# mitroitskii/crosscoder-model-diff-replication

Hardware: AMD Instinct MI355X
Metric: activations/sec per train step (fwd+bwd+Adam), 2x2304->16384; % bf16 MFMA peak (higher is better)
Workload: dtype bf16; 1 GPU; crosscoder train step 2x2304->16384, batch 4096; global_batch=4096, n_models=2, d_model=2304, dict_size=16384, parallelism=latent1

## Files before the change

crosscoder-model-diff-replication_amd/_lib.py:

```python
import contextlib
import ctypes
import os

_HERE = os.path.dirname(os.path.abspath(__file__))
LIB_PATH = os.path.join(_HERE, "libcrosscoder_hip.so")
DEBUG_LIB_PATH = os.path.join(_HERE, "libcrosscoder_hip_dbg.so")
DEFAULT_PP_MASK = 7
_INT_SETTERS = ("cc_debug_set_pp_mask", "cc_debug_set_pp_fast", "cc_debug_set_dec_one_launch",
                "cc_debug_set_wave_sync", "cc_debug_set_epi_store", "cc_debug_set_q4", "cc_debug_set_adam_ref")
DEBUG_SETTERS = _INT_SETTERS + ("cc_debug_adam_prims", "cc_debug_adam_redone")

CC_BF16 = 1
CC_F32 = 2
CC_LAYOUT_KC = 0
CC_LAYOUT_MN = 1

_p = ctypes.c_void_p


class LossTailJob(ctypes.Structure):
    _fields_ = [("colsum_acts", ctypes.c_void_p), ("tn", ctypes.c_void_p), ("h", ctypes.c_int64),
                ("l1_part", ctypes.c_void_p), ("row_part", ctypes.c_void_p), ("ncb", ctypes.c_int64),
                ("l0_part", ctypes.c_void_p), ("n_l0", ctypes.c_int64), ("ev", ctypes.c_void_p),
                ("ev_a", ctypes.c_void_p), ("ev_b", ctypes.c_void_p), ("scalars", ctypes.c_void_p),
                ("l1l0_out", ctypes.c_void_p), ("host_out", ctypes.c_void_p), ("seq", ctypes.c_uint32),
                ("B", ctypes.c_int64), ("n", ctypes.c_int64), ("counter", ctypes.c_void_p)]


class ColsumJob(ctypes.Structure):
    _fields_ = [("part", ctypes.c_void_p), ("rows", ctypes.c_int64), ("cols", ctypes.c_int64), ("ld", ctypes.c_int64),
                ("scale", ctypes.c_float), ("out", ctypes.c_void_p)]
_i64 = ctypes.c_int64
_i = ctypes.c_int
_f = ctypes.c_float
_d = ctypes.c_double

SIGNATURES = {
    "cc_version": (_i, []),
    "cc_strerror": (ctypes.c_char_p, [_i]),
    "cc_col_part_rows": (_i64, [_i64]),
    "cc_wave_parts": (_i64, [_i64, _i64]),
    "cc_wgrad_parts": (_i64, [_i64, _i64, _i]),
    "cc_prep_part_rows": (_i64, [_i64]),
    "cc_loss_part_rows": (_i64, [_i64]),
    "cc_loss_col_blocks": (_i64, [_i64]),
    "cc_loss_scalars_len": (_i64, [_i64]),
# ... 52 lines not shown
                                    ctypes.c_double, _i64, _i64, _p, _p, _i, _p]),
    "cc_gather_rows": (_i, [_p, _i64, _p, _p, _i64, _i64, _p]),
    "cc_fold_scaling": (_i, [_p, _p, _p, _p, _i64, _i64, _i64, _i, _p]),
    "cc_decoder_stats": (_i, [_p, _i64, _i64, _i64, _i, _p, _p, _p, _p]),
    "cc_latent_stats_max_k": (_i, []),
    "cc_latent_stats_update": (_i, [_p, _i64, _i64, _i64, _i, _p, _i64, _i, _p, _p, _p, _p, _p, _p]),
    "cc_topk_part_rows": (_i64, [_i64, _i64]),
    "cc_topk_l0_parts": (_i64, [_i64, _i64]),
    "cc_topk_rows": (_i, [_p, _i64, _i64, _i64, _i, _i, _p, _p, _p, _p, _p, _p]),
    "cc_batch_topk_part_rows": (_i64, [_i64, _i64]),
    "cc_batch_topk_l0_parts": (_i64, [_i64, _i64]),
    "cc_batch_topk_ws_bytes": (_i64, [_i64, _i64, _i, _i]),
    "cc_batch_topk": (_i, [_p, _i64, _i64, _i64, _i, _p, _i64, _p, _p, _p, _p, _p, _p, _f, _p, _i64, _p]),
    "cc_threshold_mask": (_i, [_p, _i64, _i64, _i64, _i, _p, _p, _p, _p, _p, _p, _p]),
    "cc_adam_step": (_i, [_p, _p, _p, _p, _i64, _p, _d, _d, _d, _d, _i64, _i64, _i, _p]),
    "cc_adam_step_clip": (_i, [_p, _p, _p, _p, _i64, _p, _i, _f, _i, _p, _d, _d, _d, _d, _i64, _i64, _i, _p]),
    "cc_adam_dec_norms": (_i, [_p, _p, _p, _p, _i64, _p, _p, _i, _f, _i, _d, _d, _d, _d, _i64, _i64, _p, _i64, _i64, _i,
                               _p, _p]),
    "cc_adam_capped_blocks": (_i64, [_i64, _i64]),
    "cc_auxk_rows": (_i, [_p, _i64, _i64, _i64, _i, _i, _p, _i64, _p, _p, _p]),
    "cc_dead_update": (_i, [_p, _p, _i64, _i64, _i64, _i64, _p, _p, _p, _p]),
    "cc_auxk_part_floats": (_i64, [_i64, _i64]),
    "cc_auxk_loss": (_i, [_p, _p, _p, _p, _p, _p, _p, _p, _f, _i64, _i64, _i, _p]),
    "cc_add_rows": (_i, [_p, _p, _i64, _i64, _i64, _i, _p]),
    "cc_jumprelu_part_rows": (_i64, [_i64, _i64]),
    "cc_jumprelu_l0_parts": (_i64, [_i64, _i64]),
    "cc_jumprelu_mask": (_i, [_p, _i64, _i64, _i64, _i, _p, _f, _p, _p, _p, _p, _p]),
    "cc_jumprelu_bwd": (_i, [_p, _p, _i64, _i64, _i64, _i, _p, _f, _f, _p, _p, _p]),
}

# ... 78 lines not shown
```

crosscoder-model-diff-replication_amd/buffer.py:

```python
import numpy as np
import torch
import torch.distributed as dist
import tqdm

from . import ops
from .crosscoder import DTYPES



def _coll_device(group, default):
    if dist.get_backend(group) == "nccl":
        return torch.device("cuda", torch.cuda.current_device())
    return default


def _src(group, r):
    return dist.get_global_rank(group, r) if group is not None and group != dist.group.WORLD else r


def fingerprint(buf, factor):
    words = buf.reshape(buf.shape[0], -1).view(torch.int16)
    rows = words.shape[0]
    total = torch.zeros((), dtype=torch.int64, device=buf.device)
    step = 4096
# ... 110 lines not shown
            spare = torch.empty_like(self.buffer)
        self.gather_rows(self.buffer, perm, out=spare)
        self._spare, self.buffer = self.buffer, spare
        self.refresh_count += 1

    def next_raw(self):
        B = self.cfg["batch_size"]
        out = self.buffer[self.buffer_pointer: self.buffer_pointer + B]
        self.buffer_pointer += B
        if self.buffer_pointer > self.buffer.shape[0] // 2 - B:
            if out.dtype != torch.float32:
                out = out.clone()
            self.refresh()
        return out, self.normalisation_factor


class SyntheticBuffer(_BufferProtocol):

    RAW_SCALES = (1 / 0.2759, 1 / 0.2442, 1 / 0.31, 1 / 0.27)

    def __init__(self, cfg, rows, n_models=2, seed=0, device=None):
        device = device or cfg["device"]
        self.cfg = cfg
        self.dtype = DTYPES[cfg["enc_dtype"]]
        d = cfg["d_in"]
        g = torch.Generator(device=device).manual_seed(seed)
        scales = torch.tensor([self.RAW_SCALES[i % 4] for i in range(n_models)], device=device)
        buf = torch.empty(rows, n_models, d, dtype=self.dtype, device=device)
        chunk = 65536
        for r0 in range(0, rows, chunk):
# ... 1 lines not shown
            z = torch.randn(r1 - r0, n_models, d, generator=g, device=device)
            buf[r0:r1] = (z * scales[None, :, None]).to(self.dtype)
        self.buffer = buf
        sample = buf[: min(rows, 4096)].float()
        f = [(d ** 0.5) / sample[:, i].norm(dim=-1).mean().item() for i in range(n_models)]
        self.normalisation_factor = torch.tensor(f, device=device, dtype=self.dtype)
        self.buffer_pointer = 0

    def next_raw(self):
        B = self.cfg["batch_size"]
        if self.buffer_pointer + B > self.buffer.shape[0]:
            self.buffer_pointer = 0
        out = self.buffer[self.buffer_pointer: self.buffer_pointer + B]
        self.buffer_pointer += B
        return out, self.normalisation_factor
```

crosscoder-model-diff-replication_amd/csrc/step_kernels.hip:

```cpp
#include "cc_common.h"

#include <cfloat>
#include <cmath>

namespace cc {

#include "grad_tail.h"

constexpr int PREP_ROWS = 64;
constexpr int LOSS_ROWS = 32;
constexpr int LOSS_COLS = 512;

typedef __attribute__((address_space(3))) bf16x4 lds_bf16x4_s;
CC_DEV void tile_put8(char* lds, int r, int chunk, const float v[8]) {
  bf16x8 b;
#pragma unroll
  for (int j = 0; j < 8; ++j) b[j] = (short)f2bf(v[j]);
  *(bf16x8*)(lds + r * 1024 + ((chunk ^ (r & 7)) << 4)) = b;
}
template <int R, bool NT = false>
CC_DEV void tile_store_transposed(const char* lds, void* out_t, int64_t ldt, int64_t col0, int ncols, int64_t row0,
                                  int nrows) {
  constexpr int RQ = R / 32;
  const int lane = threadIdx.x & 63, wave = threadIdx.x >> 6;
  const int g = lane >> 4, i = lane & 15, q = i >> 2, p = i & 3;
  for (int it = wave; it < 32 * RQ; it += 4) {
    const int cg = it / RQ, rb = (it % RQ) * 32 + g * 8;
    const int ca = cg * 16 + 4 * p, c = cg * 16 + i;
    const int l0 = rb + q, l1 = rb + 4 + q;
    const bf16x4 v0 = __builtin_amdgcn_ds_read_tr16_b64_v4i16(
        (lds_bf16x4_s*)(lds + l0 * 1024 + (((ca >> 3) ^ (l0 & 7)) << 4) + (ca & 4) * 2));
    const bf16x4 v1 = __builtin_amdgcn_ds_read_tr16_b64_v4i16(
        (lds_bf16x4_s*)(lds + l1 * 1024 + (((ca >> 3) ^ (l1 & 7)) << 4) + (ca & 4) * 2));
    if (c < ncols && rb < nrows) {
      const bf16x8 v = bf16x8{v0[0], v0[1], v0[2], v0[3], v1[0], v1[1], v1[2], v1[3]};
      bf16x8* dst = (bf16x8*)((bf16_t*)out_t + (col0 + c) * ldt + row0 + rb);
      if constexpr (NT) __builtin_nontemporal_store(v, dst);
      else *dst = v;
    }
  }
}

template <int DIN, int DF, int DT, bool TR = false>
__global__ __launch_bounds__(256) void prep_kernel(const void* __restrict__ x_in, const void* __restrict__ factor,
                                                   void* __restrict__ x_out, float* __restrict__ colsum_part, int B,
                                                   int n, int d, void* __restrict__ x_t) {
  __shared__ __attribute__((aligned(16))) char lds[TR ? 32 * 1024 : 4 * 512 * 4];
  float(*red)[512] = (float(*)[512])lds;
// ... 43 lines not shown
#pragma unroll
        for (int j = 0; j < 8; ++j) v[u][j] = Elem<DT>::round(v[u][j] * f);
        store8<DT>(x_out, (int64_t)r * K + col, v[u]);
#pragma unroll
        for (int j = 0; j < 8; ++j) cs[j] += v[u][j];
      }
    }
  }
  if (!colsum_part) return;
#pragma unroll
  for (int j = 0; j < 8; ++j) red[wave][lane * 8 + j] = cs[j];
  __syncthreads();
  for (int i = threadIdx.x; i < 512; i += 256) {
    int c = blockIdx.x * 512 + i;
    if (c < K) colsum_part[(int64_t)blockIdx.y * K + c] = ((red[0][i] + red[1][i]) + red[2][i]) + red[3][i];
  }
}

template <int DT>
__global__ __launch_bounds__(256) void reduce_rows_kernel(const RedSeg a) {
  __shared__ float red[4][RED_COLS];
  reduce_rows_phase1(a, blockIdx.x, threadIdx.x, red);
  __syncthreads();
  reduce_rows_phase2<DT>(a, blockIdx.x, threadIdx.x, red);
}

template <int DT>
__global__ __launch_bounds__(256) void dec_norms_kernel(const void* __restrict__ W, float* __restrict__ norms,
                                                        float* __restrict__ total, float* __restrict__ inv_norms, int h,
                                                        int n, int d) {
// ... 434 lines not shown
  n.col += n.dcol;
  if (n.col >= ld) {
    n.col -= ld;
    ++n.row;
  }
}
CC_DEV void norm_part_store(const AdamArgs& a, const NormPos& n, float q) {
  if (a.norm_part && n.row < a.norm_rows) {
    q = block8_sum(q);
    if ((threadIdx.x & 7) == 0) a.norm_part[(int64_t)n.row * (a.norm_ld >> 6) + (n.col >> 6)] = q;
  }
}

constexpr int ADAM_U = 1;

template <int DT, int U, bool LO>
__global__ __launch_bounds__(256) void adam_bulk_kernel(const AdamArgs a, int64_t nchunks) {
  const int64_t c0 = (int64_t)blockIdx.x * 256 * U + threadIdx.x;
  constexpr bool PN = false, SN = true;
  if constexpr (DT == CC_BF16) {
    bf16x8 p[U], g[U], m[U], v[U];
#pragma unroll
    for (int u = 0; u < U; ++u) {
      const int64_t c = c0 + u * 256;
      if (c < nchunks) {
        p[u] = ld_bf16x8<PN>(a.p, c * 8); g[u] = ld_bf16x8<SN>(a.g, c * 8); m[u] = ld_bf16x8<SN>(a.m, c * 8);
        v[u] = ld_bf16x8<SN>(a.v, c * 8);
      }
    }
    const float coef = adam_coef_block(a);
    if (coef < 0.f) return;
#pragma unroll
    for (int u = 0; u < U; ++u) {
      const int64_t c = c0 + u * 256;
      if (c < nchunks) {
        adam_chunk_bf16<LO>(a, coef, c * 8, p[u], g[u], m[u], v[u]);
        st_bf16x8<PN>(a.p, c * 8, p[u]); st_bf16x8<SN>(a.m, c * 8, m[u]); st_bf16x8<SN>(a.v, c * 8, v[u]);
      }
    }
    return;
  }
  float p[U][8], g[U][8], m[U][8], v[U][8];
#pragma unroll
  for (int u = 0; u < U; ++u) {
    const int64_t c = c0 + u * 256;
    if (c < nchunks) {
      ld8<DT, PN>(a.p, c * 8, p[u]); ld8<DT, SN>(a.g, c * 8, g[u]); ld8<DT, SN>(a.m, c * 8, m[u]);
      ld8<DT, SN>(a.v, c * 8, v[u]);
    }
  }
  const float coef = adam_coef_block(a);
  if (coef < 0.f) return;
#pragma unroll
  for (int u = 0; u < U; ++u) {
    const int64_t c = c0 + u * 256;
    if (c < nchunks) {
#pragma unroll
      for (int j = 0; j < 8; ++j) adam_elem<DT>(a, coef, p[u][j], g[u][j], m[u][j], v[u][j]);
      st8<DT, PN>(a.p, c * 8, p[u]); st8<DT, SN>(a.m, c * 8, m[u]); st8<DT, SN>(a.v, c * 8, v[u]);
    }
  }
}

template <int DT, bool LO>
__global__ __launch_bounds__(256) void adam_kernel(const AdamArgs a) {
  using E = Elem<DT>;
  const float coef = adam_coef(a);
  const int64_t stride = (int64_t)gridDim.x * 256 * 8;
  const int64_t numel = coef < 0.f ? 0 : a.numel;
  const int64_t i0 = ((int64_t)blockIdx.x * 256 + threadIdx.x) * 8;
  NormPos np = norm_pos(a, i0, stride);
  for (int64_t i = i0; i < numel; i += stride, norm_pos_next(np, a.norm_ld)) {
    const bool full = i + 8 <= a.numel;
    if constexpr (DT == CC_BF16) {
      if (full) {
        bf16x8 p = ld_bf16x8<true>(a.p, i), g = ld_bf16x8<true>(a.g, i), m = ld_bf16x8<true>(a.m, i),
// ... 515 lines not shown
}

int cc_adam_step_clip(void* p, const void* g, void* m, void* v, int64_t numel, const float* sums, int nparams,
                      float max_norm, int emulate_bf16, float* clip_out, double lr, double beta1, double beta2,
                      double eps, int64_t step, int64_t max_blocks, int dtype, void* stream) {
  if (!p || !g || !m || !v || !sums) return CC_ERR_NULL;
  if (numel <= 0 || step <= 0 || nparams <= 0 || nparams > 6) return CC_ERR_SHAPE;
  if (!al16(p) || !al16(g) || !al16(m) || !al16(v)) return CC_ERR_ALIGN;
  AdamArgs a = adam_args(p, g, m, v, numel, nullptr, lr, beta1, beta2, eps, step);
  a.clip_sums = sums;
  a.clip_np = nparams;
  a.clip_emulate = emulate_bf16;
  a.clip_max_norm = max_norm;
  a.clip_out = clip_out;
  return adam_launch(a, max_blocks, dtype, (hipStream_t)stream);
}

int64_t cc_adam_capped_blocks(int64_t numel, int64_t max_blocks) {
  return numel > 0 && max_blocks > 0 ? adam_capped_blocks(numel, max_blocks) : 0;
}

int cc_adam_dec_norms(void* p, const void* g, void* m, void* v, int64_t numel, const float* coef, const float* sums,
                      int nparams, float max_norm, int emulate_bf16, double lr, double beta1, double beta2,
                      double eps, int64_t step, int64_t max_blocks, float* norm_part, int64_t h, int64_t K, int dtype,
                      uint32_t* done_ctr, void* stream) {
  if (!p || !g || !m || !v || !norm_part || (!coef && !sums)) return CC_ERR_NULL;
  if (done_ctr && max_blocks <= 0) return CC_ERR_SHAPE;
  if (numel <= 0 || step <= 0 || h <= 0 || K <= 0 || K % 64 || h * K > numel || h * K >= ((int64_t)1 << 31))
    return CC_ERR_SHAPE;
  if (sums && (nparams <= 0 || nparams > 6)) return CC_ERR_SHAPE;
// ... 140 lines not shown
```

crosscoder-model-diff-replication_amd/engine.py:

```python
import contextlib

import torch

from . import _hip, ops

TIMER = None


def _span(name):
    return TIMER.span(name) if TIMER is not None else contextlib.nullcontext()


DYNAMIC_TILES = True


LOSS_TAIL_IN_G3 = True


G2_WAITS_IN_KERNEL = True


def _tile_ctr(ws, k):
    return ws.tile_ctr[k] if DYNAMIC_TILES else None


def padded_dims(h, d):
    return -(-h // 8) * 8, -(-d // 8) * 8


class Arena:

    def __init__(self, h, n, d, dtype, device, data=None, ref=None):
        self.h, self.n, self.d = h, n, d
        self.h_ref, self.d_ref = ref if ref is not None else (h, d)
# ... 163 lines not shown
        self.sq_off = [0]
        for s in sizes:
            self.sq_off.append(self.sq_off[-1] + s)
        self.sq = E(self.sq_off[-1])
        self.clip_out = E(8)
        self.tile_sum = E(ops.wgrad_tile_sums(h, K))
        ops.wgrad_clock(self.tile_sum).zero_()
        self.tile_ctr = torch.zeros(3, ops.TILE_CTR_WORDS, dtype=torch.int32, device=device)
        self.clip_ready = False
        self.acts_pending = False
        self.tail_ctr = torch.zeros(2, dtype=torch.int32, device=device)
        self.adam_done = torch.zeros(8, dtype=torch.int32, device=device)
        self.adam_done_target = 0
        self.wait_err = None
        self.norms_token = None
        self.busy = None

    def next_slot(self):
        self._slot ^= 1
        self.acts_colpart, self.l0_part, self.colsum_acts = self._slots[self._slot]

    def sq_slice(self, i):
        return self.sq[self.sq_off[i]:self.sq_off[i + 1]]


def transposed_wgrad(B, K, h, dtype):
    return bool(ops.lib().cc_transposed_ok(B, K, h, ops.dtype_code(dtype)))


def _norms_token(P):
# ... 21 lines not shown
    if ws.norms_fin_pending:
        ws.norms_fin_pending = False
        with _span("dec_norms"):
            ops.dec_norms_finalize(ws.norm_part, ws.h, ws.n, ws.d, ws.norms, ws.tn, ws.inv_norms)


def decoder_norms(ws, P):
    if getattr(ws, "norms_token", None) == _norms_token(P):
        ws.norms_token = None
        return
    ws.norms_token = None
    _decoder_derived(ws, P)


def forward(ws, P, x_in, factor=None, grad_scale=None, want_grad=True, loss=True, finalize=True, bt_threshold=None,
            aux=None, theta=None):
    B, n, d, h, K = ws.B, ws.n, ws.d, ws.h, ws.K
    ws.next_slot()
    with _span("prep"):
        ops.prep_input(x_in, factor, ws.dtype, out=ws.x, colsum_part=ws.x_colpart, out_t=ws.x_t)
    fused = bool(loss and ws.fused_ncb)
    x_job = ops.colsum_job(ws.x_colpart, ws.x_colpart.shape[0], K, 1.0 / B, ws.x_mean) if ws.tr else None
    with _span("G1_encode"):
        if ws.tr:
            ops.encode_fwd_t(ws.x, P.W_enc_hk, P.b_enc, ws.acts, ws.acts_t, True, colsum_part=ws.acts_colpart,
                             l0_part=ws.l0_part, mask_bits=ws.mask_bits, tile_ctr=_tile_ctr(ws, 0), pre=x_job)
        elif ws.topk is None and ws.batch_topk is None and ws.jumprelu is None:
            ops.encode_fwd(ws.x, P.W_enc_hk, P.b_enc, ws.acts, True, colsum_part=ws.acts_colpart,
                           l0_part=ws.l0_part)
        else:
            ops.encode_fwd(ws.x, P.W_enc_hk, P.b_enc, ws.acts, True)
    if aux is not None:
        with _span("auxk_rows"):
            ops.auxk_rows(ws.acts, h, ws.k_aux, aux[0], aux[1], out=ws.aux_acts, row_count=ws.aux_row_count)
    if ws.topk is not None:
# ... 292 lines not shown
        ops.wgrad_dec(ws.acts_full, ws.g_recon_full, P.W_dec_hk, ws.inv_norms, ws.colsum_acts, l1_scale, G.W_dec_hk,
                      ws.sq_slice(1), n, d)
    with _span("G5_wgrad_enc"):
        ops.wgrad_enc(ws.g_pre, ws.x, G.W_enc_hk, ws.sq_slice(0))
    ops.grad_tail(ws.gpre_colpart_full, G.b_enc, ws.sq_slice(2), loss_colpart(ws), G.b_dec_flat, ws.sq_slice(3), ws.sq,
                  ws.sq_off, clip, ws.dtype == torch.bfloat16, ws.clip_out, ws.tail_ctr[1:2])
    ws.clip_ready = True


DEC_ADAM_BLOCKS = 256
DEC_SIDE_ROWS = 1.0
DEC_ADAM_BESIDE_G1 = True
SERIAL_DEC_BLOCKS = 0


def clip_and_adam(ws, P, G, M, V, lr, beta1, beta2, eps, step, max_norm=1.0, side_stream=None, extra=None):
    emulate = clip_emulation(ws, len(ws.sq_off) - 1)
    if not ws.clip_ready:
        ops.clip_finalize(ws.sq, ws.sq_off, max_norm, emulate, ws.clip_out)
    ws.clip_ready = False
    adam(ws, P, G, M, V, lr, beta1, beta2, eps, step, side_stream, extra=extra)


def adam(ws, P, G, M, V, lr, beta1, beta2, eps, step, side_stream=None, clip_sums=None, extra=None):
    P.wait_pending()
    P.updates += 1
    coef = ws.clip_out[0:1]
    emulate = ws.dtype == torch.bfloat16
    if extra is not None:
        if clip_sums is not None:
            raise ValueError("extra parameters take the step's own coefficient")
        with _span("adam_theta"):
            ops.adam_step(*extra, coef, lr, beta1, beta2, eps, step)

    def step_(p, g, m, v, max_blocks=0, clip_out=None):
        if clip_sums is None:
            ops.adam_step(p, g, m, v, coef, lr, beta1, beta2, eps, step, max_blocks=max_blocks)
        else:
            ops.adam_step_clip(p, g, m, v, clip_sums[0], clip_sums[1], emulate, lr, beta1, beta2, eps, step,
                               max_blocks=max_blocks, clip_out=clip_out)

    if side_stream is None:
        with _span("adam"):
            step_(P.data, G.data, M.data, V.data, clip_out=ws.clip_out)
        return
    dev = P.data.device
    with _span("adam"):
        step_(P.enc_part(), G.enc_part(), M.enc_part(), V.enc_part(), clip_out=ws.clip_out)
    if not DEC_ADAM_BESIDE_G1 and ws.W_dec_t is None and ws.norm_part is not None:
        dec = [A.dec_part() for A in (P, G, M, V)]
        with _span("adam_dec"):
            ops.adam_dec_norms(*dec, ws.h, ws.K, lr, beta1, beta2, eps, step, ws.norm_part,
                               coef=coef if clip_sums is None else None, clip_sums=clip_sums, emulate=emulate,
                               max_blocks=SERIAL_DEC_BLOCKS)
        ws.norms_token = _norms_token(P)
        ws.norms_fin_pending = True
        return
    enc_done = _hip.DeviceEvent().record(torch.cuda.current_stream(dev))
    ws.fork_events[1] = enc_done
    with torch.cuda.stream(side_stream):
        enc_done.wait(side_stream)
        if ws.W_dec_t is None and ws.norm_part is not None:
            K, nblk = ws.K, ws.K // 64
            hs = min(ws.h, int(ws.h * DEC_SIDE_ROWS) // 8 * 8)
            dec = [A.dec_part() for A in (P, G, M, V)]
            kw = dict(coef=coef if clip_sums is None else None, clip_sums=clip_sums, emulate=emulate)
            hp = (lr, beta1, beta2, eps, step)
            target = None
            if hs > 0:
                with _span("adam_dec"):
                    nb = ops.adam_dec_norms(*(t[:hs * K] for t in dec), hs, K, *hp, ws.norm_part[:hs * nblk],
                                            max_blocks=DEC_ADAM_BLOCKS, done_ctr=ws.adam_done, **kw)
                ws.adam_done_target = (ws.adam_done_target + nb) & 0xFFFFFFFF
                target = ws.adam_done_target
            done = _hip.DeviceEvent().record(side_stream)

            def rest(kernel_wait=False):
                cur = torch.cuda.current_stream(dev)
                with _span("adam_dec_rest"):
                    if ws.h > hs:
                        ops.adam_dec_norms(*(t[hs * K:] for t in dec), ws.h - hs, K, *hp, ws.norm_part[hs * nblk:],
                                           **kw)
                    else:
                        step_(*(t[hs * K:] for t in dec))
                ws.norms_fin_pending = True
                if kernel_wait and target is not None:
                    P.pending = done
                    return ws.adam_done, target
                done.wait(cur)
                return None

            ws.norms_token = _norms_token(P)
            P.pending_rest = rest
            P.pending = None
            return
        else:
            with _span("adam_dec"):
                step_(P.dec_part(), G.dec_part(), M.dec_part(), V.dec_part(), max_blocks=DEC_ADAM_BLOCKS)
            norms_for_next(ws, P)
# ... 3 lines not shown
```

crosscoder-model-diff-replication_amd/ops.py:

```python
import ctypes

import torch

from . import _lib
from ._lib import CC_BF16, CC_F32, CC_LAYOUT_KC, CC_LAYOUT_MN

_DT = {torch.bfloat16: CC_BF16, torch.float32: CC_F32}


def dtype_code(dtype):
    try:
        return _DT[dtype]
    except KeyError:
        raise TypeError(f"crosscoder_amd supports bf16 and fp32 storage, got {dtype}") from None


def lib():
    return _lib.load()


def _stream(t):
    if t.device.type != "cuda":
        raise RuntimeError(
            f"crosscoder_amd kernels run on a ROCm GPU; got a tensor on {t.device} "
# ... 417 lines not shown
        _ptr(sq_dec), _ptr(g_preT), _ptr(xT), _ptr(grad_enc), _ptr(sq_enc), B, h, n, d, _ptr(gpre_colpart),
        gpre_colpart.shape[0], _ptr(g_b_enc), _ptr(sq_b_enc), _ptr(loss_colpart), loss_colpart.shape[0], _ptr(g_b_dec),
        _ptr(sq_b_dec), _ptr(sq), arr, len(offsets) - 1, int(zero_mask), _ptr(out), _ptr(counter), _ptr(tile_sum),
        _ctr(tile_ctr), _vptr(abort_ptr), dtype_code(actsT.dtype), _stream(actsT)))


def clip_finalize(sq, offsets, max_norm, emulate_bf16, out):
    arr = (ctypes.c_int64 * len(offsets))(*[int(o) for o in offsets])
    check(lib().cc_clip_finalize(_ptr(sq), arr, len(offsets) - 1, max_norm, int(emulate_bf16), _ptr(out),
                                 _stream(sq)))


def adam_step(p, g, m, v, coef, lr, beta1, beta2, eps, step, max_blocks=0):
    check(lib().cc_adam_step(_ptr(p), _ptr(g), _ptr(m), _ptr(v), p.numel(), _ptr(coef), lr, beta1, beta2, eps,
                             int(step), int(max_blocks), dtype_code(p.dtype), _stream(p)))


def adam_step_clip(p, g, m, v, sums, max_norm, emulate_bf16, lr, beta1, beta2, eps, step, max_blocks=0,
                   clip_out=None):
    check(lib().cc_adam_step_clip(_ptr(p), _ptr(g), _ptr(m), _ptr(v), p.numel(), _ptr(sums), sums.numel(),
                                  float(max_norm), int(emulate_bf16), _ptr(clip_out), lr, beta1, beta2, eps, int(step),
                                  int(max_blocks), dtype_code(p.dtype), _stream(p)))


def gather_rows(src, perm, out=None):
    _contig(src, "src")
    if perm.dtype != torch.int64 or perm.device != src.device:
        raise ValueError("perm must be an int64 tensor on the source's device")
    rows = perm.numel()
    if out is None:
# ... 254 lines not shown
```

crosscoder-model-diff-replication_amd/trainer.py:

```python
import torch
import tqdm

from . import _hip, engine
from .buffer import Buffer
from .crosscoder import CrossCoder


def reference_loss(l2, l1, l1c, dtype):
    t = torch.tensor(l2, dtype=torch.float32) + l1c * torch.tensor(l1, dtype=dtype)
    return t.item()


def jumprelu_loss(loss, l0, l0c):
    return (torch.tensor(loss, dtype=torch.float32) + l0c * torch.tensor(l0, dtype=torch.float32)).item()


def rounded(v, dtype):
    return float(torch.tensor(v, dtype=dtype)) if dtype != torch.float32 else float(torch.tensor(v))


class FusedAdam:

    def __init__(self, cc, lr, betas, eps=1e-8):
        a = cc.arena()
# ... 115 lines not shown
        if self.auxk is None or ws is None:
            raise ValueError("auxk_state(): no AuxK step has run")
        torch.cuda.synchronize(ws.x.device)
        hr = self.crosscoder.d_hidden
        sc = ws.auxk_scalars.cpu()
        active = ws.aux_active
        return {"aux_acts": ws.aux_acts[:, :hr] if active else torch.zeros_like(ws.aux_acts[:, :hr]),
                "dead": ws.was_dead[:hr].bool(), "row_count": ws.aux_row_count if active else None,
                "den": float(sc[1]) if active else 0.0, "auxk_loss": float(sc[0]) if active else 0.0,
                "dead_latents": int(ws.dead_count)}

    def _launch_step(self, host, seq):
        cc = self.crosscoder
        raw, factor = self.buffer.next_raw()
        raw = cc.pad_input(raw)
        ws = cc._workspace(raw.shape[0], step=True)
        P = cc.arena()
        opt = self.optimizer
        side = self._side_stream()
        aux_on = self.auxk is not None and self._dead_count > 0
        engine.forward(ws, P, raw, factor if getattr(self.buffer, "normalize", True) else None, finalize=False,
                       bt_threshold=(cc.threshold, cc.threshold_beta) if ws.batch_topk is not None else None,
                       aux=(self._since_fired(), self.auxk[2]) if aux_on else None,
                       theta=cc.theta() if ws.jumprelu is not None else None)
        if self.latent_stats is not None:
            self.latent_stats.update_from_acts(ws.acts, row0=self.step_counter * self.cfg["batch_size"])
        if self.auxk is not None:
            engine.auxk_forward(ws, P, self._since_fired(), cc.d_hidden, self.auxk[2], self.auxk[0], aux_on, host=host)
        engine.loss_finalize_with_g3(ws, side, host=host, seq=seq)
        l1c = self.get_l1_coeff()
        l0c = None
        if ws.jumprelu is not None:
            l0c = self.get_l0_coeff()
            engine.backward(ws, P, opt.grads, l1c, clip=1.0, l0_coeff=l0c, theta_grad=opt.theta_grad)
        elif aux_on:
            engine.backward_auxk(ws, P, opt.grads, l1c, clip=1.0)
        else:
            engine.backward(ws, P, opt.grads, l1c, clip=1.0)
        g = opt.param_groups[0]
        opt.t += 1
        b1, b2 = g["betas"]
        engine.clip_and_adam(ws, P, opt.grads, opt.exp_avg, opt.exp_avg_sq, g["lr"], b1, b2, g["eps"], opt.t,
                             side_stream=side,
                             extra=(ws.theta, opt.theta_grad, opt.theta_m, opt.theta_v) if l0c is not None else None)
        self.scheduler.step()
        self._last_l1c = l1c
        self._last_l0c = l0c
        self._last_ws = ws
        self._last_aux_on = aux_on

    def _side_stream(self):
        if self._side is None:
            self._side = torch.cuda.Stream(device=self.crosscoder.arena().data.device)
        return self._side

    def synchronize(self):
        self.crosscoder.arena().wait_pending()
        self._check_abort()
# ... 68 lines not shown
```

include/crosscoder_hip.h:

```cpp
#ifndef CROSSCODER_HIP_H
#define CROSSCODER_HIP_H

#include <stdint.h>

#ifdef __cplusplus
extern "C" {
#endif
#pragma GCC visibility push(default)

#define CC_BF16 1
#define CC_F32 2

#define CC_LAYOUT_KC 0
#define CC_LAYOUT_MN 1

enum {
  CC_OK = 0,
  CC_ERR_NULL = 1,
  CC_ERR_DTYPE = 2,
  CC_ERR_SHAPE = 3,
  CC_ERR_ALIGN = 4,
  CC_ERR_TOO_LARGE = 5,
  CC_ERR_HIP_BASE = 1000
};
// ... 159 lines not shown
                         const void* xT, void* grad_W_enc, float* sq_enc, int64_t B, int64_t h, int64_t n, int64_t d,
                         const float* gpre_colpart, int64_t R_enc, void* g_b_enc, float* sq_b_enc,
                         const float* loss_colpart, int64_t R_dec, void* g_b_dec, float* sq_b_dec, const float* sq,
                         const int64_t* off, int nparams, int zero_mask, float* out, uint32_t* counter, float* tile_sum,
                         uint32_t* tile_ctr, const uint32_t* abort, int dtype, void* stream);
int cc_grad_tail_sums(const float* gpre_colpart, int64_t R_enc, int64_t h, void* g_b_enc, float* sq_b_enc,
                      const float* loss_colpart, int64_t R_dec, int64_t K, void* g_b_dec, float* sq_b_dec, int dtype,
                      const float* sq, const int64_t* off, int nparams, int zero_mask, float* out, uint32_t* counter,
                      void* stream);

int cc_segment_sums(const float* sq, const int64_t* off, int nparams, int zero_mask, float* out, void* stream);

int cc_adam_step(void* p, const void* g, void* m, void* v, int64_t numel, const float* coef, double lr,
                 double beta1, double beta2, double eps, int64_t step, int64_t max_blocks, int dtype, void* stream);

int cc_adam_step_clip(void* p, const void* g, void* m, void* v, int64_t numel, const float* sums, int nparams,
                      float max_norm, int emulate_bf16, float* clip_out, double lr, double beta1, double beta2,
                      double eps, int64_t step, int64_t max_blocks, int dtype, void* stream);


int cc_transpose_b16(const void* src, int64_t rows, int64_t cols, int64_t ld_src, void* dst, int64_t ld_dst,
                     void* stream);

int64_t cc_dec_norms_part_floats(int64_t h, int64_t n, int64_t d);
int cc_transpose_dec_norms(const void* W_dec, int64_t h, int64_t n, int64_t d, void* W_dec_t, float* part,
                           float* norms, float* total, float* inv_norms, void* stream);

int cc_dec_norms_finalize(const float* part, int64_t h, int64_t n, int64_t d, float* norms, float* total,
                          float* inv_norms, void* stream);

// ... 66 lines not shown
```

Before: 1.647 million activations/s.

## Fuse next-batch input prep into encoder Adam kernel and move b_dec Adam to side

Adds a combined kernel that, in one launch, runs the encoder Adam update alongside the input prep (scale, bf16 cast, transpose and column partial sums) for the next batch. The next batch is taken from a new buffer peek. On the next forward, the prepped buffers are swapped in when a token matching pointer, version, tag and stream is found, so the separate prep launch is skipped. It also folds the remaining decoder/bias Adam work into the side-stream decoder Adam call when the side covers every row. The aim is to hide prep's memory traffic under the bandwidth-bound Adam pass and to cut launches. The cost is extra buffers and a cache whose validity rests on the token checks.

```diff
diff --git a/crosscoder-model-diff-replication_amd/_lib.py b/crosscoder-model-diff-replication_amd/_lib.py
--- a/crosscoder-model-diff-replication_amd/_lib.py
+++ b/crosscoder-model-diff-replication_amd/_lib.py
@@ -30,6 +30,14 @@
 class ColsumJob(ctypes.Structure):
     _fields_ = [("part", ctypes.c_void_p), ("rows", ctypes.c_int64), ("cols", ctypes.c_int64), ("ld", ctypes.c_int64),
                 ("scale", ctypes.c_float), ("out", ctypes.c_void_p)]
+
+
+class PrepJob(ctypes.Structure):
+    _fields_ = [("x_in", ctypes.c_void_p), ("in_dtype", ctypes.c_int), ("factor", ctypes.c_void_p),
+                ("factor_dtype", ctypes.c_int), ("x_out", ctypes.c_void_p), ("x_t", ctypes.c_void_p),
+                ("colsum_part", ctypes.c_void_p), ("B", ctypes.c_int64), ("n", ctypes.c_int64), ("d", ctypes.c_int64)]
+
+
 _i64 = ctypes.c_int64
 _i = ctypes.c_int
 _f = ctypes.c_float
@@ -112,6 +120,7 @@
     "cc_batch_topk": (_i, [_p, _i64, _i64, _i64, _i, _p, _i64, _p, _p, _p, _p, _p, _p, _f, _p, _i64, _p]),
     "cc_threshold_mask": (_i, [_p, _i64, _i64, _i64, _i, _p, _p, _p, _p, _p, _p, _p]),
     "cc_adam_step": (_i, [_p, _p, _p, _p, _i64, _p, _d, _d, _d, _d, _i64, _i64, _i, _p]),
+    "cc_adam_step_prep": (_i, [_p, _p, _p, _p, _i64, _p, _d, _d, _d, _d, _i64, _i, _p, _p]),
     "cc_adam_step_clip": (_i, [_p, _p, _p, _p, _i64, _p, _i, _f, _i, _p, _d, _d, _d, _d, _i64, _i64, _i, _p]),
     "cc_adam_dec_norms": (_i, [_p, _p, _p, _p, _i64, _p, _p, _i, _f, _i, _d, _d, _d, _d, _i64, _i64, _p, _i64, _i64, _i,
                                _p, _p]),
diff --git a/crosscoder-model-diff-replication_amd/buffer.py b/crosscoder-model-diff-replication_amd/buffer.py
--- a/crosscoder-model-diff-replication_amd/buffer.py
+++ b/crosscoder-model-diff-replication_amd/buffer.py
@@ -148,6 +148,13 @@
             self.refresh()
         return out, self.normalisation_factor
 
+    def peek_raw(self):
+        B = self.cfg["batch_size"]
+        p = self.buffer_pointer
+        if p + B > self.buffer.shape[0] // 2 - B and self.buffer.dtype == torch.float32:
+            return None
+        return self.buffer[p: p + B], self.normalisation_factor
+
 
 class SyntheticBuffer(_BufferProtocol):
 
@@ -179,3 +186,8 @@
         out = self.buffer[self.buffer_pointer: self.buffer_pointer + B]
         self.buffer_pointer += B
         return out, self.normalisation_factor
+
+    def peek_raw(self):
+        B = self.cfg["batch_size"]
+        p = self.buffer_pointer if self.buffer_pointer + B <= self.buffer.shape[0] else 0
+        return self.buffer[p: p + B], self.normalisation_factor
diff --git a/crosscoder-model-diff-replication_amd/csrc/step_kernels.hip b/crosscoder-model-diff-replication_amd/csrc/step_kernels.hip
--- a/crosscoder-model-diff-replication_amd/csrc/step_kernels.hip
+++ b/crosscoder-model-diff-replication_amd/csrc/step_kernels.hip
@@ -18,20 +18,21 @@
   for (int j = 0; j < 8; ++j) b[j] = (short)f2bf(v[j]);
   *(bf16x8*)(lds + r * 1024 + ((chunk ^ (r & 7)) << 4)) = b;
 }
-template <int R, bool NT = false>
+template <int R, bool NT = false, int PITCH = 1024>
 CC_DEV void tile_store_transposed(const char* lds, void* out_t, int64_t ldt, int64_t col0, int ncols, int64_t row0,
                                   int nrows) {
   constexpr int RQ = R / 32;
+  constexpr int NCG = PITCH / 32;
   const int lane = threadIdx.x & 63, wave = threadIdx.x >> 6;
   const int g = lane >> 4, i = lane & 15, q = i >> 2, p = i & 3;
-  for (int it = wave; it < 32 * RQ; it += 4) {
+  for (int it = wave; it < NCG * RQ; it += 4) {
     const int cg = it / RQ, rb = (it % RQ) * 32 + g * 8;
     const int ca = cg * 16 + 4 * p, c = cg * 16 + i;
     const int l0 = rb + q, l1 = rb + 4 + q;
     const bf16x4 v0 = __builtin_amdgcn_ds_read_tr16_b64_v4i16(
-        (lds_bf16x4_s*)(lds + l0 * 1024 + (((ca >> 3) ^ (l0 & 7)) << 4) + (ca & 4) * 2));
+        (lds_bf16x4_s*)(lds + l0 * PITCH + (((ca >> 3) ^ (l0 & 7)) << 4) + (ca & 4) * 2));
     const bf16x4 v1 = __builtin_amdgcn_ds_read_tr16_b64_v4i16(
-        (lds_bf16x4_s*)(lds + l1 * 1024 + (((ca >> 3) ^ (l1 & 7)) << 4) + (ca & 4) * 2));
+        (lds_bf16x4_s*)(lds + l1 * PITCH + (((ca >> 3) ^ (l1 & 7)) << 4) + (ca & 4) * 2));
     if (c < ncols && rb < nrows) {
       const bf16x8 v = bf16x8{v0[0], v0[1], v0[2], v0[3], v1[0], v1[1], v1[2], v1[3]};
       bf16x8* dst = (bf16x8*)((bf16_t*)out_t + (col0 + c) * ldt + row0 + rb);
@@ -105,6 +106,65 @@
   for (int i = threadIdx.x; i < 512; i += 256) {
     int c = blockIdx.x * 512 + i;
     if (c < K) colsum_part[(int64_t)blockIdx.y * K + c] = ((red[0][i] + red[1][i]) + red[2][i]) + red[3][i];
+  }
+}
+
+constexpr int PREPN_COLS = 128, PREPN_LDS = 32 * PREPN_COLS * 2;
+template <int DIN, int DF>
+CC_DEV void prep_block_narrow(char* lds, int bx, int by, const void* __restrict__ x_in,
+                              const void* __restrict__ factor, void* __restrict__ x_out,
+                              float* __restrict__ colsum_part, int B, int n, int d, void* __restrict__ x_t) {
+  constexpr int PITCH = PREPN_COLS * 2;
+  const int K = n * d;
+  const int ch = threadIdx.x & 15, slot = threadIdx.x >> 4;
+  const int col = bx * PREPN_COLS + ch * 8;
+  const int r0 = by * PREP_ROWS;
+  const int scol = threadIdx.x & 127, sw = threadIdx.x >> 7;
+  float acc[2] = {0.f, 0.f};
+  float f = 1.f;
+  if (factor && col < K) f = Elem<DF>::load((const typename Elem<DF>::T*)factor + col / d);
+  for (int half = 0; half < 2; ++half) {
+    const int base = r0 + 32 * half;
+    if (base >= B) break;
+    const int nr = B - base < 32 ? B - base : 32;
+    if (col < K) {
+      float v[2][8];
+#pragma unroll
+      for (int k = 0; k < 2; ++k)
+        if (slot + 16 * k < nr) load8<DIN>(x_in, (int64_t)(base + slot + 16 * k) * K + col, v[k]);
+#pragma unroll
+      for (int k = 0; k < 2; ++k) {
+        const int r = slot + 16 * k;
+        if (r >= nr) break;
+#pragma unroll
+        for (int j = 0; j < 8; ++j) v[k][j] = Elem<CC_BF16>::round(v[k][j] * f);
+        store8<CC_BF16>(x_out, (int64_t)(base + r) * K + col, v[k]);
+        bf16x8 b;
+#pragma unroll
+        for (int j = 0; j < 8; ++j) b[j] = (short)f2bf(v[k][j]);
+        *(bf16x8*)(lds + r * PITCH + ((ch ^ (r & 7)) << 4)) = b;
+      }
+    }
+    __syncthreads();
+    tile_store_transposed<32, true, PITCH>(lds, x_t, B, (int64_t)bx * PREPN_COLS, K - bx * PREPN_COLS, base, nr);
+#pragma unroll
+    for (int c = 0; c < 2; ++c)
+#pragma unroll
+      for (int k = 0; k < 8; ++k) {
+        const int r = sw + 2 * c + 4 * k;
+        if (r < nr)
+          acc[c] += bf2f(*(const bf16_t*)(lds + r * PITCH + (((scol >> 3) ^ (r & 7)) << 4) + (scol & 7) * 2));
+      }
+    __syncthreads();
+  }
+  if (!colsum_part) return;
+  float(*red)[PREPN_COLS] = (float(*)[PREPN_COLS])lds;
+  red[sw][scol] = acc[0];
+  red[sw + 2][scol] = acc[1];
+  __syncthreads();
+  if (threadIdx.x < PREPN_COLS) {
+    const int c = bx * PREPN_COLS + threadIdx.x, i = threadIdx.x;
+    if (c < K) colsum_part[(int64_t)by * K + c] = ((red[0][i] + red[1][i]) + red[2][i]) + red[3][i];
   }
 }
 
@@ -569,30 +629,40 @@
 
 constexpr int ADAM_U = 1;
 
+constexpr bool ADAM_PN = false, ADAM_SN = true;
+template <int U, bool LO, bool BLOCK_COEF = true>
+CC_DEV void adam_bulk_bf16(const AdamArgs& a, int64_t nchunks, int64_t block) {
+  constexpr bool PN = ADAM_PN, SN = ADAM_SN;
+  const int64_t c0 = block * 256 * U + threadIdx.x;
+  bf16x8 p[U], g[U], m[U], v[U];
+#pragma unroll
+  for (int u = 0; u < U; ++u) {
+    const int64_t c = c0 + u * 256;
+    if (c < nchunks) {
+      p[u] = ld_bf16x8<PN>(a.p, c * 8); g[u] = ld_bf16x8<SN>(a.g, c * 8); m[u] = ld_bf16x8<SN>(a.m, c * 8);
+      v[u] = ld_bf16x8<SN>(a.v, c * 8);
+    }
+  }
+  float coef;
+  if constexpr (BLOCK_COEF) coef = adam_coef_block(a);
+  else coef = a.coef ? *a.coef : 1.f;
+  if (coef < 0.f) return;
+#pragma unroll
+  for (int u = 0; u < U; ++u) {
+    const int64_t c = c0 + u * 256;
+    if (c < nchunks) {
+      adam_chunk_bf16<LO>(a, coef, c * 8, p[u], g[u], m[u], v[u]);
+      st_bf16x8<PN>(a.p, c * 8, p[u]); st_bf16x8<SN>(a.m, c * 8, m[u]); st_bf16x8<SN>(a.v, c * 8, v[u]);
+    }
+  }
+}
+
 template <int DT, int U, bool LO>
 __global__ __launch_bounds__(256) void adam_bulk_kernel(const AdamArgs a, int64_t nchunks) {
   const int64_t c0 = (int64_t)blockIdx.x * 256 * U + threadIdx.x;
-  constexpr bool PN = false, SN = true;
+  constexpr bool PN = ADAM_PN, SN = ADAM_SN;
   if constexpr (DT == CC_BF16) {
-    bf16x8 p[U], g[U], m[U], v[U];
-#pragma unroll
-    for (int u = 0; u < U; ++u) {
-      const int64_t c = c0 + u * 256;
-      if (c < nchunks) {
-        p[u] = ld_bf16x8<PN>(a.p, c * 8); g[u] = ld_bf16x8<SN>(a.g, c * 8); m[u] = ld_bf16x8<SN>(a.m, c * 8);
-        v[u] = ld_bf16x8<SN>(a.v, c * 8);
-      }
-    }
-    const float coef = adam_coef_block(a);
-    if (coef < 0.f) return;
-#pragma unroll
-    for (int u = 0; u < U; ++u) {
-      const int64_t c = c0 + u * 256;
-      if (c < nchunks) {
-        adam_chunk_bf16<LO>(a, coef, c * 8, p[u], g[u], m[u], v[u]);
-        st_bf16x8<PN>(a.p, c * 8, p[u]); st_bf16x8<SN>(a.m, c * 8, m[u]); st_bf16x8<SN>(a.v, c * 8, v[u]);
-      }
-    }
+    adam_bulk_bf16<U, LO>(a, nchunks, blockIdx.x);
     return;
   }
   float p[U][8], g[U][8], m[U][8], v[U][8];
@@ -615,6 +685,26 @@
       st8<DT, PN>(a.p, c * 8, p[u]); st8<DT, SN>(a.m, c * 8, m[u]); st8<DT, SN>(a.v, c * 8, v[u]);
     }
   }
+}
+
+struct PrepJob {
+  const void* x_in;
+  const void* factor;
+  void* x_out;
+  float* colsum_part;
+  void* x_t;
+  int B, n, d;
+  int gx, blocks;
+};
+template <bool LO, int DIN, int DF>
+__global__ __launch_bounds__(256) void adam_bulk_prep_kernel(const AdamArgs a, int64_t nchunks, const PrepJob j) {
+  __shared__ __attribute__((aligned(16))) char lds[PREPN_LDS];
+  if ((int)blockIdx.x < j.blocks) {
+    prep_block_narrow<DIN, DF>(lds, blockIdx.x % j.gx, blockIdx.x / j.gx, j.x_in, j.factor, j.x_out, j.colsum_part,
+                               j.B, j.n, j.d, j.x_t);
+    return;
+  }
+  adam_bulk_bf16<ADAM_U, LO, false>(a, nchunks, (int64_t)blockIdx.x - j.blocks);
 }
 
 template <int DT, bool LO>
@@ -1160,6 +1250,42 @@
   a.clip_max_norm = max_norm;
   a.clip_out = clip_out;
   return adam_launch(a, max_blocks, dtype, (hipStream_t)stream);
+}
+
+int cc_adam_step_prep(void* p, const void* g, void* m, void* v, int64_t numel, const float* coef, double lr,
+                      double beta1, double beta2, double eps, int64_t step, int dtype, const cc_prep_job* prep,
+                      void* stream) {
+  if (!prep)
+    return cc_adam_step(p, g, m, v, numel, coef, lr, beta1, beta2, eps, step, 0, dtype, stream);
+  if (!p || !g || !m || !v || !prep->x_in || !prep->x_out || !prep->x_t) return CC_ERR_NULL;
+  if (dtype != CC_BF16) return CC_ERR_DTYPE;
+  if (numel <= 0 || numel % 8 || step <= 0) return CC_ERR_SHAPE;
+  if (!al16(p) || !al16(g) || !al16(m) || !al16(v)) return CC_ERR_ALIGN;
+  const int64_t B = prep->B, n = prep->n, d = prep->d;
+  if (B <= 0 || n <= 0 || d <= 0 || d % 8 || B % 8 || B > INT32_MAX || n * d > INT32_MAX) return CC_ERR_SHAPE;
+  if (!al16(prep->x_in) || !al16(prep->x_out) || !al16(prep->x_t)) return CC_ERR_ALIGN;
+  if (prep->factor && prep->factor_dtype != CC_BF16 && prep->factor_dtype != CC_F32) return CC_ERR_DTYPE;
+  if (prep->in_dtype != CC_BF16 && prep->in_dtype != CC_F32) return CC_ERR_DTYPE;
+  const AdamArgs a = adam_args(p, g, m, v, numel, coef, lr, beta1, beta2, eps, step);
+  const int64_t nchunks = numel / 8;
+  const int64_t gx = (n * d + PREPN_COLS - 1) / PREPN_COLS, pblocks = gx * cc_prep_part_rows(B);
+  const int64_t blocks = pblocks + (nchunks + 256 * ADAM_U - 1) / (256 * ADAM_U);
+  if (blocks > INT32_MAX) return CC_ERR_SHAPE;
+  const PrepJob j = {prep->x_in, prep->factor, prep->x_out, prep->colsum_part, prep->x_t,
+                     (int)B,     (int)n,       (int)d,      (int)gx,           (int)pblocks};
+  hipStream_t st = (hipStream_t)stream;
+  const bool fb = prep->factor && prep->factor_dtype == CC_BF16;
+#define ADAM_PREP(DI, DF)                                                                                        \
+  ADAM_LO(a, hipLaunchKernelGGL((adam_bulk_prep_kernel<LO_, DI, DF>), dim3((unsigned)blocks), dim3(256), 0, st, a, \
+                                nchunks, j))
+  if (prep->in_dtype == CC_BF16) {
+    if (fb) ADAM_PREP(CC_BF16, CC_BF16); else ADAM_PREP(CC_BF16, CC_F32);
+  } else {
+    if (fb) ADAM_PREP(CC_F32, CC_BF16); else ADAM_PREP(CC_F32, CC_F32);
+  }
+#undef ADAM_PREP
+  CC_LAUNCH_CHECK();
+  return CC_OK;
 }
 
 int64_t cc_adam_capped_blocks(int64_t numel, int64_t max_blocks) {
diff --git a/crosscoder-model-diff-replication_amd/engine.py b/crosscoder-model-diff-replication_amd/engine.py
--- a/crosscoder-model-diff-replication_amd/engine.py
+++ b/crosscoder-model-diff-replication_amd/engine.py
@@ -18,6 +18,18 @@
 
 
 G2_WAITS_IN_KERNEL = True
+
+
+PREP_IN_ADAM = True
+
+
+BDEC_IN_SIDE_ADAM = True
+
+
+def _prep_token(x_in, factor, tag):
+    f = None if factor is None else (factor.data_ptr(), factor.dtype, tuple(factor.shape), factor._version)
+    return (x_in.data_ptr(), x_in.dtype, tuple(x_in.shape), x_in.stride(), x_in._version, f, tag,
+            torch.cuda.current_stream(x_in.device).cuda_stream)
 
 
 def _tile_ctr(ws, k):
@@ -211,6 +223,8 @@
         self.adam_done_target = 0
         self.wait_err = None
         self.norms_token = None
+        self.prep_token = None
+        self.x_next = None
         self.busy = None
 
     def next_slot(self):
@@ -262,11 +276,15 @@
 
 
 def forward(ws, P, x_in, factor=None, grad_scale=None, want_grad=True, loss=True, finalize=True, bt_threshold=None,
-            aux=None, theta=None):
+            aux=None, theta=None, prep_tag=None):
     B, n, d, h, K = ws.B, ws.n, ws.d, ws.h, ws.K
     ws.next_slot()
-    with _span("prep"):
-        ops.prep_input(x_in, factor, ws.dtype, out=ws.x, colsum_part=ws.x_colpart, out_t=ws.x_t)
+    prepped, ws.prep_token = ws.prep_token, None
+    if prepped is not None and prepped == _prep_token(x_in, factor, prep_tag):
+        (ws.x, ws.x_t, ws.x_colpart), ws.x_next = ws.x_next, (ws.x, ws.x_t, ws.x_colpart)
+    else:
+        with _span("prep"):
+            ops.prep_input(x_in, factor, ws.dtype, out=ws.x, colsum_part=ws.x_colpart, out_t=ws.x_t)
     fused = bool(loss and ws.fused_ncb)
     x_job = ops.colsum_job(ws.x_colpart, ws.x_colpart.shape[0], K, 1.0 / B, ws.x_mean) if ws.tr else None
     with _span("G1_encode"):
@@ -589,15 +607,17 @@
 SERIAL_DEC_BLOCKS = 0
 
 
-def clip_and_adam(ws, P, G, M, V, lr, beta1, beta2, eps, step, max_norm=1.0, side_stream=None, extra=None):
+def clip_and_adam(ws, P, G, M, V, lr, beta1, beta2, eps, step, max_norm=1.0, side_stream=None, extra=None,
+                  next_batch=None):
     emulate = clip_emulation(ws, len(ws.sq_off) - 1)
     if not ws.clip_ready:
         ops.clip_finalize(ws.sq, ws.sq_off, max_norm, emulate, ws.clip_out)
     ws.clip_ready = False
-    adam(ws, P, G, M, V, lr, beta1, beta2, eps, step, side_stream, extra=extra)
-
-
-def adam(ws, P, G, M, V, lr, beta1, beta2, eps, step, side_stream=None, clip_sums=None, extra=None):
+    adam(ws, P, G, M, V, lr, beta1, beta2, eps, step, side_stream, extra=extra, next_batch=next_batch)
+
+
+def adam(ws, P, G, M, V, lr, beta1, beta2, eps, step, side_stream=None, clip_sums=None, extra=None,
+         next_batch=None):
     P.wait_pending()
     P.updates += 1
     coef = ws.clip_out[0:1]
@@ -620,8 +640,21 @@
             step_(P.data, G.data, M.data, V.data, clip_out=ws.clip_out)
         return
     dev = P.data.device
+    enc = [A.enc_part() for A in (P, G, M, V)]
+    ride = None
+    if (PREP_IN_ADAM and next_batch is not None and clip_sums is None and enc[0].numel() % 8 == 0
+            and tuple(next_batch[0].shape) == (ws.B, ws.n, ws.d) and next_batch[0].device == dev
+            and ops.prep_job_ok(next_batch[0], next_batch[1], ws.dtype, ws.x_t)):
+        ride = _prep_token(*next_batch)
     with _span("adam"):
-        step_(P.enc_part(), G.enc_part(), M.enc_part(), V.enc_part(), clip_out=ws.clip_out)
+        if ride is not None:
+            if ws.x_next is None:
+                ws.x_next = tuple(torch.empty_like(t) for t in (ws.x, ws.x_t, ws.x_colpart))
+            ops.adam_step_prep(*enc, coef, lr, beta1, beta2, eps, step,
+                               ops.prep_job(next_batch[0], next_batch[1], ws.x_next[0], ws.x_next[2], ws.x_next[1]))
+        else:
+            step_(*enc, clip_out=ws.clip_out)
+    ws.prep_token = ride
     if not DEC_ADAM_BESIDE_G1 and ws.W_dec_t is None and ws.norm_part is not None:
         dec = [A.dec_part() for A in (P, G, M, V)]
         with _span("adam_dec"):
@@ -639,12 +672,14 @@
             K, nblk = ws.K, ws.K // 64
             hs = min(ws.h, int(ws.h * DEC_SIDE_ROWS) // 8 * 8)
             dec = [A.dec_part() for A in (P, G, M, V)]
+            side_bias = BDEC_IN_SIDE_ADAM and hs == ws.h
+            side_part = dec if side_bias else [t[:hs * K] for t in dec]
             kw = dict(coef=coef if clip_sums is None else None, clip_sums=clip_sums, emulate=emulate)
             hp = (lr, beta1, beta2, eps, step)
             target = None
             if hs > 0:
                 with _span("adam_dec"):
-                    nb = ops.adam_dec_norms(*(t[:hs * K] for t in dec), hs, K, *hp, ws.norm_part[:hs * nblk],
+                    nb = ops.adam_dec_norms(*side_part, hs, K, *hp, ws.norm_part[:hs * nblk],
                                             max_blocks=DEC_ADAM_BLOCKS, done_ctr=ws.adam_done, **kw)
                 ws.adam_done_target = (ws.adam_done_target + nb) & 0xFFFFFFFF
                 target = ws.adam_done_target
@@ -652,12 +687,13 @@
 
             def rest(kernel_wait=False):
                 cur = torch.cuda.current_stream(dev)
-                with _span("adam_dec_rest"):
-                    if ws.h > hs:
-                        ops.adam_dec_norms(*(t[hs * K:] for t in dec), ws.h - hs, K, *hp, ws.norm_part[hs * nblk:],
-                                           **kw)
-                    else:
-                        step_(*(t[hs * K:] for t in dec))
+                if not side_bias:
+                    with _span("adam_dec_rest"):
+                        if ws.h > hs:
+                            ops.adam_dec_norms(*(t[hs * K:] for t in dec), ws.h - hs, K, *hp, ws.norm_part[hs * nblk:],
+                                               **kw)
+                        else:
+                            step_(*(t[hs * K:] for t in dec))
                 ws.norms_fin_pending = True
                 if kernel_wait and target is not None:
                     P.pending = done
diff --git a/crosscoder-model-diff-replication_amd/ops.py b/crosscoder-model-diff-replication_amd/ops.py
--- a/crosscoder-model-diff-replication_amd/ops.py
+++ b/crosscoder-model-diff-replication_amd/ops.py
@@ -455,6 +455,31 @@
 def adam_step(p, g, m, v, coef, lr, beta1, beta2, eps, step, max_blocks=0):
     check(lib().cc_adam_step(_ptr(p), _ptr(g), _ptr(m), _ptr(v), p.numel(), _ptr(coef), lr, beta1, beta2, eps,
                              int(step), int(max_blocks), dtype_code(p.dtype), _stream(p)))
+
+
+def prep_job_ok(x_in, factor, dtype, out_t):
+    return (out_t is not None and dtype == torch.bfloat16 and x_in.dim() == 3 and x_in.shape[0] % 8 == 0
+            and x_in.shape[2] % 8 == 0 and x_in.dtype in _DT and x_in.is_contiguous() and x_in.data_ptr() % 16 == 0
+            and (factor is None or factor.dtype in _DT))
+
+
+def prep_job(x_in, factor, out, colsum_part, out_t):
+    B, n, d = x_in.shape
+    _contig(x_in, "x")
+    if out.shape != (B, n * d) or out.dtype != torch.bfloat16 or not out.is_contiguous():
+        raise ValueError("out must be a contiguous bf16 [B, n*d] tensor")
+    if out_t.shape != (n * d, B) or out_t.dtype != torch.bfloat16 or not out_t.is_contiguous():
+        raise ValueError("out_t must be a contiguous bf16 [n*d, B] tensor")
+    fdt = dtype_code(factor.dtype) if factor is not None else CC_F32
+    return ctypes.byref(_lib.PrepJob(x_in.data_ptr(), dtype_code(x_in.dtype),
+                                     factor.data_ptr() if factor is not None else None, fdt, out.data_ptr(),
+                                     out_t.data_ptr(), colsum_part.data_ptr() if colsum_part is not None else None,
+                                     B, n, d))
+
+
+def adam_step_prep(p, g, m, v, coef, lr, beta1, beta2, eps, step, prep):
+    check(lib().cc_adam_step_prep(_ptr(p), _ptr(g), _ptr(m), _ptr(v), p.numel(), _ptr(coef), lr, beta1, beta2, eps,
+                                  int(step), dtype_code(p.dtype), prep, _stream(p)))
 
 
 def adam_step_clip(p, g, m, v, sums, max_norm, emulate_bf16, lr, beta1, beta2, eps, step, max_blocks=0,
diff --git a/crosscoder-model-diff-replication_amd/trainer.py b/crosscoder-model-diff-replication_amd/trainer.py
--- a/crosscoder-model-diff-replication_amd/trainer.py
+++ b/crosscoder-model-diff-replication_amd/trainer.py
@@ -153,12 +153,14 @@
         cc = self.crosscoder
         raw, factor = self.buffer.next_raw()
         raw = cc.pad_input(raw)
+        normalize = getattr(self.buffer, "normalize", True)
+        tag = getattr(self.buffer, "refresh_count", 0)
         ws = cc._workspace(raw.shape[0], step=True)
         P = cc.arena()
         opt = self.optimizer
         side = self._side_stream()
         aux_on = self.auxk is not None and self._dead_count > 0
-        engine.forward(ws, P, raw, factor if getattr(self.buffer, "normalize", True) else None, finalize=False,
+        engine.forward(ws, P, raw, factor if normalize else None, finalize=False, prep_tag=tag,
                        bt_threshold=(cc.threshold, cc.threshold_beta) if ws.batch_topk is not None else None,
                        aux=(self._since_fired(), self.auxk[2]) if aux_on else None,
                        theta=cc.theta() if ws.jumprelu is not None else None)
@@ -179,8 +181,12 @@
         g = opt.param_groups[0]
         opt.t += 1
         b1, b2 = g["betas"]
+        peek = getattr(self.buffer, "peek_raw", None) if engine.PREP_IN_ADAM else None
+        nxt = peek() if peek is not None and cc._dp == cc.cfg["d_in"] else None
+        if nxt is not None:
+            nxt = (nxt[0], nxt[1] if normalize else None, getattr(self.buffer, "refresh_count", 0))
         engine.clip_and_adam(ws, P, opt.grads, opt.exp_avg, opt.exp_avg_sq, g["lr"], b1, b2, g["eps"], opt.t,
-                             side_stream=side,
+                             side_stream=side, next_batch=nxt,
                              extra=(ws.theta, opt.theta_grad, opt.theta_m, opt.theta_v) if l0c is not None else None)
         self.scheduler.step()
         self._last_l1c = l1c
diff --git a/include/crosscoder_hip.h b/include/crosscoder_hip.h
--- a/include/crosscoder_hip.h
+++ b/include/crosscoder_hip.h
@@ -197,6 +197,21 @@
 int cc_adam_step(void* p, const void* g, void* m, void* v, int64_t numel, const float* coef, double lr,
                  double beta1, double beta2, double eps, int64_t step, int64_t max_blocks, int dtype, void* stream);
 
+typedef struct cc_prep_job {
+  const void* x_in;
+  int in_dtype;
+  const void* factor;
+  int factor_dtype;
+  void* x_out;
+  void* x_t;
+  float* colsum_part;
+  int64_t B, n, d;
+} cc_prep_job;
+
+int cc_adam_step_prep(void* p, const void* g, void* m, void* v, int64_t numel, const float* coef, double lr,
+                      double beta1, double beta2, double eps, int64_t step, int dtype, const cc_prep_job* prep,
+                      void* stream);
+
 int cc_adam_step_clip(void* p, const void* g, void* m, void* v, int64_t numel, const float* sums, int nparams,
                       float max_norm, int emulate_bf16, float* clip_out, double lr, double beta1, double beta2,
                       double eps, int64_t step, int64_t max_blocks, int dtype, void* stream);
```

New measurement: 1.664 million activations/s (median of 6 runs). 1.01x the previous value.
